# LanaSina/evolutionary_illusion_generator

Hardware: AMD Instinct MI355X
Metric: genome fitness evals/sec at 256x256, pop=256 (higher is better)
Workload: dtype f32; 1 GPU; neat_configs/circles.txt colour pop=256, 256x256, PredNet 3,48,96,192, 21 steps, LK + rotation-symmetry score; global_pop=256, genomes_per_gpu=256, device_batch=256, structure=Circles

## Files before the change

evolutionary_illusion_generator_amd/csrc/conv_mfma.h:

```cpp
#pragma once
#include <hip/hip_runtime.h>
#include <stdint.h>

#include <type_traits>

#ifndef EIG_PRO_PRIO
#define EIG_PRO_PRIO 1
#endif
#ifndef EIG_EPI_PRIO
#define EIG_EPI_PRIO 0
#endif
#ifndef EIG_KLOOP_PRIO
#define EIG_KLOOP_PRIO 0
#endif
#ifndef EIG_S8
#define EIG_S8 16
#endif
#ifndef EIG_ABLATE
#define EIG_ABLATE 0
#endif

namespace eig {

typedef float f32x4 __attribute__((ext_vector_type(4)));

enum { EPI_RAW = 0, EPI_LSTM = 1, EPI_CONVA = 2, EPI_CONVP = 3, EPI_LSTM_PACKED = 4, EPI_UP4 = 5, EPI_UP4C = 6 };
constexpr int epi_taps(int epi) { return (epi == EPI_UP4 || epi == EPI_UP4C) ? 4 : 9; }

struct ConvSrc {
    const float* ptr;
    int C;
    int Cpad;
    int _reserved;
    int Ct;
};

struct ConvArgs {
    ConvSrc src[3];
    int nsrc;
    int H, W, B;
    int tilesX, tilesY;
    int n_nblk;
    int nwalk, nparts;
    unsigned mg[3];
    int krows;
    const float* wpk;
    int Cout;
    int clip;
    const float* bias;
    float* c_state;
    float* h_out;
    const float* peep;
    const float* P;
    float* E;
    float* Pout;
    const uint8_t* img;
    long long img_bstride;
    float* E0;
    uint8_t* frame;
    long long frame_bstride;
    int requant;
    int tile_map;
    float* raw;
    const float* acc_init;
    const float* up_src;
    int up_C;
    int up_kb;
    const float* zeros;
    unsigned long long* dbg;
};

__device__ __forceinline__ float det_expf_core(float x)
{
    const float n = rintf(x * 1.44269504088896341f);
    float r = fmaf(n, -0.693359375f, x);
    r = fmaf(n, 2.12194440e-4f, r);
    float p = 1.9875691500e-4f;
    p = fmaf(p, r, 1.3981999507e-3f);
    p = fmaf(p, r, 8.3334519073e-3f);
    p = fmaf(p, r, 4.1665795894e-2f);
    p = fmaf(p, r, 1.6666665459e-1f);
    p = fmaf(p, r, 5.0000001201e-1f);
    const float r2 = r * r;
    const float y = fmaf(p, r2, r) + 1.0f;
    const float s = __int_as_float(((int)n + 127) << 23);
    return y * s;
}
__device__ __forceinline__ float det_expf(float x)
{
    x = fminf(x, 80.0f);
    x = fmaxf(x, -80.0f);
    return det_expf_core(x);
}
#ifndef EIG_GATE_ORDER
#define EIG_GATE_ORDER 1
#endif
__device__ __forceinline__ float det_tanhf(float x);
#if EIG_GATE_ORDER
__device__ __forceinline__ float det_sigmoidf(float x) { return det_tanhf(x * 0.5f) * 0.5f + 0.5f; }
#else
__device__ __forceinline__ float det_sigmoidf(float x) { return 1.0f / (1.0f + det_expf(-x)); }
#endif
__device__ __forceinline__ float det_tanhf(float x)
{
    float ax = fabsf(x);
    if (ax < 0.625f) {
        const float z = x * x;
        float p = -5.70498872745e-3f;
        p = fmaf(p, z, 2.06390887954e-2f);
        p = fmaf(p, z, -5.37397155531e-2f);
        p = fmaf(p, z, 1.33314422036e-1f);
        p = fmaf(p, z, -3.33332819422e-1f);
        const float pz = p * z;
        return fmaf(pz, x, x);
    }
    ax = fminf(ax, 10.0f);
    const float t = det_expf_core(2.0f * ax);
    const float d = t + 1.0f, rc = __builtin_amdgcn_rcpf(d);
    float q = 2.0f * rc;
    q = fmaf(fmaf(-d, q, 2.0f), rc, q);
    const float r = 1.0f - q;
    return x < 0.0f ? -r : r;
}
__device__ __forceinline__ float relu_f(float v) { return v > 0.0f ? v : 0.0f; }

__device__ __forceinline__ void lstm_cell(float zi_, float zf_, float zc_, float zo_, float bi, float bf, float bc, float bo,
                                          float cold, float pi_, float pf_, float po_, float& cn, float& hn)
{
#if EIG_GATE_ORDER
    const float zi = (zi_ + bi) + pi_ * cold;
    const float zf = (zf_ + bf) + pf_ * cold;
    const float zc = zc_ + bc;
    const float zo = (zo_ + bo) + po_ * cold;
    const float ii = det_sigmoidf(zi), ff = det_sigmoidf(zf), oo = det_sigmoidf(zo);
    float cc = det_tanhf(zc);
    cc = cc * ii;
    const float fc = ff * cold;
    cn = cc + fc;
    hn = oo * det_tanhf(cn);
#else
    float zi = zi_ + bi; zi = fmaf(pi_, cold, zi);
    float zf = zf_ + bf; zf = fmaf(pf_, cold, zf);
    const float zc = zc_ + bc;
    float zo = zo_ + bo; zo = fmaf(po_, cold, zo);
    const float ii = det_sigmoidf(zi), ff = det_sigmoidf(zf), gg = det_tanhf(zc), oo = det_sigmoidf(zo);
    const float gi = gg * ii;
    cn = fmaf(ff, cold, gi);
    hn = oo * det_tanhf(cn);
#endif
}

template <int TW, bool VEC, bool HALF = false> struct TileGeom {
    static constexpr int TH = (TW == 8) ? 8 : 16;
    static constexpr int NIMG = HALF ? 2 : 256 / (TH * TW);
    static constexpr int S = VEC ? (TW == 16 ? TW + 8 : (TW == 4 ? 12 : EIG_S8)) : TW + 2;
    static constexpr int XO = VEC ? 3 : 0;
    static constexpr int PH = TH + 2;
    static constexpr int PLANE = NIMG * PH * S;
};

#ifndef EIG_DMA_EARLY
#define EIG_DMA_EARLY 0
#endif
#ifndef EIG_KC
#define EIG_KC 8
#endif
constexpr int KC = EIG_KC;

template <int NI, int TW, bool VEC> constexpr bool conv_fast_dma() { return VEC && TW == 16 && KC == 8 && NI >= 3; }
template <int NI, int TW, bool VEC, int TAPS = 9, int NT = 256> constexpr int conv_w_floats()
{
    return (conv_fast_dma<NI, TW, VEC>() && !(NI == 4 && TAPS == 9)) ? ((KC * TAPS * NI * 4 + NT - 1) / NT) * NT * 4 : KC * TAPS * NI * 16;
}
template <int NI, int TW, bool VEC, int NT = 256, bool HALF = false> constexpr int conv_in_floats()
{
    return conv_fast_dma<NI, TW, VEC>() ? ((KC * TileGeom<TW, VEC>::PLANE / 4 + NT - 1) / NT) * NT * 4 : KC * TileGeom<TW, VEC, HALF>::PLANE;
}
template <int NI, int TW, bool VEC, int TAPS = 9, bool ONEKB = false, int NT = 256, bool HALF = false> constexpr int conv_lds_bytes()
{
    return (ONEKB ? 1 : 2) * (conv_in_floats<NI, TW, VEC, NT, HALF>() + conv_w_floats<NI, TW, VEC, TAPS, NT>()) * 4;
}

#ifndef EIG_TIMING
#define EIG_TIMING 0
#endif
#ifndef EIG_CONV_OCC
#define EIG_CONV_OCC 2
#endif
constexpr int CONV_THREADS = 256;
#ifndef EIG_W8_OCC
#define EIG_W8_OCC 4
#endif

#ifndef EIG_UP4_OCC
#define EIG_UP4_OCC 2
#endif
#ifndef EIG_ONEKB_OCC
#define EIG_ONEKB_OCC 4
#endif
template <int NI, int TW, int EPI, bool VEC, bool ONEKB = false, bool FUSE_ = false, int SPLIT = 0>
__global__ void __launch_bounds__(SPLIT == 1 ? 512 : CONV_THREADS, SPLIT ? EIG_W8_OCC : (ONEKB ? EIG_ONEKB_OCC : ((EPI == EPI_UP4 && NI == 4 && TW == 16 && VEC) ? EIG_UP4_OCC : EIG_CONV_OCC)))
conv3x3_mfma(const ConvArgs a)
{
    constexpr bool W8 = SPLIT != 0;
    constexpr bool H4 = SPLIT == 2;
    static_assert(!H4 || TW == 8 || TW == 4, "SPLIT 2: 8- or 4-wide tiles (one image per wave) only");
    static_assert(TW != 4 || (H4 && VEC && EPI != EPI_LSTM_PACKED && EPI != EPI_UP4C), "4-wide tiles: half blocks with 16-byte staging only");
    static_assert(!FUSE_, "the in-kernel chain of an unpooled source was removed in round 6 (a ConvLSTM chains it inside only in its Winograd forms)");
    static_assert(!W8 || (VEC && !ONEKB && EPI != EPI_UP4C && EPI != EPI_LSTM_PACKED), "W8: 16-byte staging, per-pixel or pooled epilogues");
    constexpr int NT = SPLIT == 1 ? 512 : CONV_THREADS;
    constexpr int NWS = H4 ? 2 : 4;
    constexpr int MI_N = W8 ? 2 : 4;
    using G = TileGeom<TW, VEC, H4>;
    constexpr int TH = G::TH, NIMG = G::NIMG, S = G::S, XO = G::XO, PH = G::PH, PLANE = G::PLANE;
    constexpr int NB = NI * 16;
    constexpr int TAPS = epi_taps(EPI);
    static_assert(EPI != EPI_UP4C || NI == 4, "EPI_UP4C: the four N-tiles are the four parity classes");
    const unsigned long long t_entry = EIG_TIMING ? __builtin_readcyclecounter() : 0;
#if EIG_PRO_PRIO
    __builtin_amdgcn_s_setprio(EIG_PRO_PRIO);
#endif
    extern __shared__ __attribute__((aligned(16))) float lds[];
    constexpr bool FAST = conv_fast_dma<NI, TW, VEC>();
    constexpr int INF = conv_in_floats<NI, TW, VEC, NT, H4>();
    constexpr int BUF = INF + conv_w_floats<NI, TW, VEC, epi_taps(EPI), NT>();

    const int tid = threadIdx.x;
    const int lane = tid & 63;
    const int wv = __builtin_amdgcn_readfirstlane(tid >> 6);
    const int ws = W8 ? (wv % NWS) : wv;
    const int ch2 = W8 ? (wv / NWS) : 0;
    const int q = lane >> 4;
    const int col = lane & 15;

    const int tiles = a.tilesX * a.tilesY;
    const int ngroups = (a.B + NIMG - 1) / NIMG;
    const int ntile = ngroups * tiles;
    const int xcd = blockIdx.x & 7, xi = blockIdx.x >> 3;
    const int nnb = (EPI == EPI_UP4) ? a.n_nblk * 4 : a.n_nblk;
    const int nbe = xi % nnb;
    const int nblk = (EPI == EPI_UP4) ? nbe >> 2 : nbe;
    const int cls = (EPI == EPI_UP4) ? nbe & 3 : 0;
    const int tlin = a.tile_map ? xcd * ((ntile + 7) >> 3) + xi / nnb : (xi / nnb) * 8 + xcd;
    if (tlin >= ntile) return;
    const int bgrp = tlin / tiles;
    const int t = tlin - bgrp * tiles;
    const int tyi = t / a.tilesX, txi = t - tyi * a.tilesX;
    const int y0 = tyi * TH, x0 = txi * TW;

    constexpr int RC = S / 4;
    constexpr int PER_C = VEC ? NIMG * PH * RC : PLANE;
    constexpr int NR = VEC ? (KC * PER_C + NT - 1) / NT : (PLANE + NT - 1) / NT;
    int sl_off[NR], sl_img[NR];
#pragma unroll
    for (int r = 0; r < NR; ++r) {
        const int p = tid + r * NT;
        int rem = VEC ? p % PER_C : p;
        constexpr int RW = VEC ? RC : S;
        const int img = rem / (PH * RW);
        rem -= img * (PH * RW);
        const int yy = rem / RW, xx = rem - yy * RW;
        const int gy = y0 + yy - 1, gx = VEC ? (x0 - 4 + 4 * xx) : (x0 + xx - 1);
        const int b = bgrp * NIMG + img;
        const bool ok = (VEC ? p < KC * PER_C : p < PLANE) && b < a.B && gy >= 0 && gy < a.H && gx >= 0 && gx < a.W;
        sl_off[r] = ok ? (VEC ? ((p / PER_C) * a.H * a.W + gy * a.W + gx) * 4 : gy * a.W + gx) : -1;
        sl_img[r] = VEC ? img : b;
    }

    constexpr int NWR = (KC * TAPS * (NB / 4) + NT - 1) / NT;
    constexpr int NIN = VEC ? NR : KC * NR;
    constexpr int NOPS = NWR + NIN;
    constexpr int NSTEP = KC * TAPS / 4;
    struct KB { int s, c0, kc; };
    const int cpad0 = a.src[0].Cpad, cpad1 = a.src[1].Cpad, cpad2 = a.src[2].Cpad;
    auto cpad_of = [&](int si) __attribute__((always_inline)) { return si == 0 ? cpad0 : (si == 1 ? cpad1 : cpad2); };
    auto kb_first = [&]() { KB k; k.s = 0; k.c0 = 0; k.kc = min(KC, cpad0); return k; };
    auto kb_next = [&](KB k) __attribute__((always_inline)) {
        k.c0 += KC;
        if (k.c0 >= cpad_of(k.s)) { k.c0 = 0; ++k.s; }
        k.kc = (k.s < a.nsrc) ? min(KC, cpad_of(k.s) - k.c0) : 0;
        return k;
    };
    const int b0 = bgrp * NIMG;
    const int nimg_here = min(NIMG, a.B - b0);
    auto make_rsrc = [&](const float* ptr, int C, int Ct) {
        const size_t plane = (size_t)(a.H * a.W);
        return __builtin_amdgcn_make_buffer_rsrc((void*)(ptr + (size_t)b0 * Ct * plane), 0, (int)(((size_t)(nimg_here - 1) * Ct + C) * plane * 4), 0x00020000);
    };
    const bool has1 = a.nsrc > 1, has2 = a.nsrc > 2;
    const __amdgpu_buffer_rsrc_t rs0 = make_rsrc(a.src[0].ptr, a.src[0].C, a.src[0].Ct);
    const __amdgpu_buffer_rsrc_t rs1 = make_rsrc(has1 ? a.src[1].ptr : a.src[0].ptr, has1 ? a.src[1].C : a.src[0].C, has1 ? a.src[1].Ct : a.src[0].Ct);
    const __amdgpu_buffer_rsrc_t rs2 = make_rsrc(has2 ? a.src[2].ptr : a.src[0].ptr, has2 ? a.src[2].C : a.src[0].C, has2 ? a.src[2].Ct : a.src[0].Ct);
    const __amdgpu_buffer_rsrc_t rsw = __builtin_amdgcn_make_buffer_rsrc((void*)(a.wpk + ((size_t)cls * a.n_nblk + nblk) * a.krows * NB), 0, a.krows * NB * 4, 0x00020000);
    auto buf_dma16 = [&](int si, float* lds_dst, int voff, int soff) {
        auto l = (__attribute__((address_space(3))) void*)lds_dst;
        if (si == 0) __builtin_amdgcn_raw_ptr_buffer_load_lds(rs0, l, 16, voff, soff, 0, 0);
        else if (si == 1) __builtin_amdgcn_raw_ptr_buffer_load_lds(rs1, l, 16, voff, soff, 0, 0);
        else __builtin_amdgcn_raw_ptr_buffer_load_lds(rs2, l, 16, voff, soff, 0, 0);
    };
    auto dma_op = [&](int j, const KB& k, int wrow, float* buf) {
        ConvSrc src;
        src.ptr = k.s == 0 ? a.src[0].ptr : (k.s == 1 ? a.src[1].ptr : a.src[2].ptr);
        src.C = k.s == 0 ? a.src[0].C : (k.s == 1 ? a.src[1].C : a.src[2].C);
        src.Cpad = cpad_of(k.s);
        src.Ct = k.s == 0 ? a.src[0].Ct : (k.s == 1 ? a.src[1].Ct : a.src[2].Ct);
        if (j < NWR) {
            const int n16 = k.kc * TAPS * (NB / 4);
            const int base = j * NT + wv * 64, ch = base + lane;
            if (ch < n16)
                __builtin_amdgcn_raw_ptr_buffer_load_lds(rsw, (__attribute__((address_space(3))) void*)(buf + INF + (size_t)base * 4), 16,
                                                         tid * 16, (wrow * NB + j * NT * 4) * 4, 0, 0);
            return;
        }
        const int chs = a.H * a.W;
        if (VEC) {
            const int r = j - NWR;
            const int p = tid + r * NT;
            const int soff = k.c0 * chs * 4;
            const bool tail = k.c0 + KC > src.C;
            if (r < NR) {
                int vo = sl_off[r < NR ? r : 0];
                if (NIMG > 1) vo = vo < 0 ? vo : vo + sl_img[r < NR ? r : 0] * src.Ct * chs * 4;
                if (tail && k.c0 + p / PER_C >= src.C) vo = -1;
                if (p < k.kc * PER_C) buf_dma16(k.s, buf + (r * NT + wv * 64) * 4, vo, soff);
            }
        } else {
            const int c = (j - NWR) / NR, r = (j - NWR) % NR;
            if (c < k.kc) {
                const bool pok = sl_off[r] >= 0;
                const int gy = pok ? sl_off[r] / a.W : 0, gx = pok ? sl_off[r] - gy * a.W : 0;
                const float* g = (pok && (k.c0 + c < src.C))
                                     ? src.ptr + ((size_t)sl_img[r] * src.Ct + k.c0 + c) * chs + gy * a.W + gx : a.zeros;
                if (tid + r * NT < PLANE)
                    __builtin_amdgcn_global_load_lds((const __attribute__((address_space(1))) void*)g,
                                                     (__attribute__((address_space(3))) void*)(buf + c * PLANE + r * NT + wv * 64), 4, 0, 0);
            }
        }
    };

    constexpr int LASTW = (NWR - 1) * NT;
    const int vw_full = tid * 16;
    const int vw_last = (LASTW + (wv & 1) * 64 + lane) * 16;
    static_assert(!FAST || NI != 4 || TAPS != 9 || (KC * 9 * (NB / 4)) % NT == 128, "FAST staging: the last weight round of NI = 4 must hold 128 chunks");
    static_assert(!FAST || TAPS != 4 || NI != 4 || (KC * 4 * (NB / 4)) % NT == 0, "FAST staging, 2x2 form: whole weight rounds");
    const int aH = a.H, aW = a.W;
    auto src_base = [&](const float* ptr, int Ct) __attribute__((always_inline)) { return ptr + (size_t)b0 * Ct * (a.H * a.W); };
    auto src_bytes = [&](int C, int Ct) __attribute__((always_inline)) { return ((nimg_here - 1) * Ct + C) * (a.H * a.W) * 4; };
    const float* const sp0 = src_base(a.src[0].ptr, a.src[0].Ct);
    const float* const sp1 = has1 ? src_base(a.src[1].ptr, a.src[1].Ct) : sp0;
    const float* const sp2 = has2 ? src_base(a.src[2].ptr, a.src[2].Ct) : sp0;
    const int sn0 = src_bytes(a.src[0].C, a.src[0].Ct);
    const int sn1 = has1 ? src_bytes(a.src[1].C, a.src[1].Ct) : sn0;
    const int sn2 = has2 ? src_bytes(a.src[2].C, a.src[2].Ct) : sn0;
    const unsigned long long su0 = (unsigned long long)sp0, sd1 = (unsigned long long)sp1 - su0, sd2 = (unsigned long long)sp2 - (unsigned long long)sp1;
    auto rsrc_of = [=](int si) __attribute__((always_inline)) {
        const unsigned long long u = su0 + (si > 0 ? sd1 : 0ull) + (si > 1 ? sd2 : 0ull);
        const int n = sn0 + (si > 0 ? sn1 - sn0 : 0) + (si > 1 ? sn2 - sn1 : 0);
        const unsigned lo = __builtin_amdgcn_readfirstlane((unsigned)u), hi = __builtin_amdgcn_readfirstlane((unsigned)(u >> 32));
        return __builtin_amdgcn_make_buffer_rsrc((void*)(((unsigned long long)hi << 32) | lo), 0, __builtin_amdgcn_readfirstlane(n), 0x00020000);
    };
    auto dma_fast = [=](int j, const KB k, const __amdgpu_buffer_rsrc_t rs_k, unsigned soff_in, unsigned soff_w, float* buf) __attribute__((always_inline)) {
        if (j < NWR) {
            const unsigned soff = soff_w;
            const bool lastw = TAPS == 9 && NI == 4 && (j == NWR - 1);
            if (SPLIT == 1 && lastw && wv >= 2) return;
            const unsigned vo = __builtin_elementwise_add_sat((unsigned)(lastw ? vw_last : vw_full + j * NT * 16), soff);
            float* dst = buf + INF + (lastw ? (LASTW + (wv & 1) * 64) * 4 : (j * NT + wv * 64) * 4);
            __builtin_amdgcn_raw_ptr_buffer_load_lds(rsw, (__attribute__((address_space(3))) void*)dst, 16, (int)vo, 0, 0, 0);
            return;
        }
        const int r = j - NWR;
        const unsigned soff = soff_in;
        const int slot = r < NR ? sl_off[r < NR ? r : 0] : -1;
        const unsigned vo = __builtin_elementwise_add_sat((unsigned)slot, soff);
        __builtin_amdgcn_raw_ptr_buffer_load_lds(rs_k, (__attribute__((address_space(3))) void*)(buf + (r * NT + wv * 64) * 4), 16, (int)vo, 0, 0, 0);
    };

    const unsigned long long t_setup = EIG_TIMING ? __builtin_readcyclecounter() : 0;
    int nkb = 0;
    for (int s = 0; s < a.nsrc; ++s) nkb += (cpad_of(s) + KC - 1) / KC;
    KB cur_kb = kb_first();
    int wrow = 0;

#pragma unroll
    for (int j = 0; j < NOPS; ++j) {
        if constexpr (FAST) dma_fast(j, cur_kb, rsrc_of(0), 0u, 0u, lds);
        else dma_op(j, cur_kb, wrow, lds);
    }

    int addrA[9];
    const int g_wy = (TW == 16) ? (col & 3) >> 1 : (TW == 4 ? 2 * (col >> 2) + ((col & 3) >> 1) : col >> 2);
    const int g_wx = (TW == 16) ? 2 * (col >> 2) + (col & 1) : (TW == 4 ? col & 1 : col & 3);
    const int g_base = ((TW == 16) ? (ws * 4 + 2 * g_wy) * S + 2 * g_wx + XO
                                   : ws * PH * S + 2 * g_wy * S + 2 * g_wx + XO)
                       + ch2 * S;
    {
#pragma unroll
        for (int s = 0; s < 9; ++s) {
            const int k = 4 * s + q;
            const int c = k / 9, tap = k - 9 * c;
            const int ky = tap / 3, kx = tap - 3 * ky;
            addrA[s] = g_base + c * PLANE + ky * S + kx;
        }
    }
    const int addr4 = g_base + ((q >> 1) + (cls >> 1)) * S + (q & 1) + (cls & 1);
    const int boff = q * NB + col * NI;

    f32x4 acc[MI_N][NI];
#pragma unroll
    for (int mi = 0; mi < MI_N; ++mi)
#pragma unroll
        for (int ni = 0; ni < NI; ++ni) acc[mi][ni] = (f32x4){0.f, 0.f, 0.f, 0.f};

    const unsigned long long t_prewait = EIG_TIMING ? __builtin_readcyclecounter() : 0;
#if EIG_KLOOP_PRIO
    __builtin_amdgcn_s_setprio(EIG_KLOOP_PRIO);
#endif
#if EIG_PRO_PRIO
    __builtin_amdgcn_s_setprio(0);
#endif
    asm volatile("s_waitcnt vmcnt(0)" ::: "memory");
    __syncthreads();

    constexpr bool HAS_UP = (EPI == EPI_LSTM || EPI == EPI_LSTM_PACKED || EPI == EPI_RAW);
    constexpr int UPV = (TW != 8) ? 2 : 1;
    constexpr int NUPL = HAS_UP ? MI_N * NI * UPV : 0;
    f32x4 upc[MI_N][HAS_UP ? NI : 1];
    const bool has_up = HAS_UP && a.acc_init != nullptr;
    int up_off[UPV];
    const float* up_base = a.acc_init;
    int up_hw = 0, up_cstride = 0;
    if (has_up) {
        const int Hs = a.H >> 1, Ws = a.W >> 1;
        up_hw = Hs * Ws;
        up_cstride = a.n_nblk * NB * up_hw;
        const int b = bgrp * NIMG + (TW == 16 ? 0 : ws);
#pragma unroll
        for (int v = 0; v < UPV; ++v) {
            const int gy0 = (TW == 16) ? y0 + 4 * ws + 2 * v : (TW == 4 ? tyi * TH + 4 * q + 2 * v : tyi * TH + 2 * q);
            const int gx0 = (TW == 16) ? x0 + 4 * q : txi * TW;
            up_off[v] = (b < a.B && gy0 < a.H && gx0 < a.W) ? ((nblk * NB + col) * up_hw + (gy0 >> 1) * Ws + (gx0 >> 1)) * 4 : 0;
        }
        const int bw = __builtin_amdgcn_readfirstlane(b);
        up_base = a.acc_init + (size_t)(bw < a.B ? bw : 0) * 4 * up_cstride;
    }
    const __amdgpu_buffer_rsrc_t rs_up = __builtin_amdgcn_make_buffer_rsrc((void*)up_base, 0, has_up ? 4 * up_cstride * 4 : 0, 0x00020000);
    auto up_load = [&](int mi, int ni, int v) __attribute__((always_inline)) {
        const int soff = (ni * 16 * up_hw + (W8 ? 2 * ch2 + mi : mi) * up_cstride) * 4;
        if constexpr (TW != 8) {
            typedef float f32x2 __attribute__((ext_vector_type(2)));
            const f32x2 t = __builtin_bit_cast(f32x2, __builtin_amdgcn_raw_buffer_load_b64(rs_up, up_off[v], soff, 0));
            upc[mi][ni][2 * v] = t[0]; upc[mi][ni][2 * v + 1] = t[1];
        } else {
            upc[mi][ni] = __builtin_bit_cast(f32x4, __builtin_amdgcn_raw_buffer_load_b128(rs_up, up_off[0], soff, 0));
        }
    };

    unsigned long long t_mfma = 0, t_wait = 0, t_bar = 0, t_all0 = EIG_TIMING ? __builtin_readcyclecounter() : 0;
    auto kiter = [&](const int kb, auto kfirst_tag) __attribute__((always_inline)) {
        const unsigned long long tk0 = EIG_TIMING ? __builtin_readcyclecounter() : 0;
        float* const cur = lds + (kb & 1) * BUF;
        float* const nxt = lds + ((kb & 1) ^ 1) * BUF;
        const KB nxt_kb = kb_next(cur_kb);
        const int wrow_nxt = wrow + cur_kb.kc * TAPS;
        const bool more_kb = (kb + 1 < nkb) && EIG_ABLATE != 1;
        const __amdgpu_buffer_rsrc_t rs_nxt = rsrc_of(nxt_kb.s);
        const unsigned soff_in_nxt = more_kb ? (unsigned)(nxt_kb.c0 * (aH * aW) * 4) : 0x80000000u;
        const unsigned soff_w_nxt = more_kb ? (unsigned)(wrow_nxt * NB * 4) : 0x80000000u;

        const float* const in_lds = cur;
        const float* const w_lds = cur + INF + boff;
        auto body = [&](auto first_tag) {
            constexpr bool FIRST = decltype(first_tag)::value;
            constexpr int PL = PLANE;
            const int* const ad = addrA;
#pragma unroll
            for (int st = 0; st < NSTEP; ++st) {
                if (FAST || (TAPS == 9 ? (st < 9 || cur_kb.kc > 4) : st < cur_kb.kc)) {
                    const int per = st / 9, s9 = st % 9;
                    float av[MI_N], bv[NI];
                    float avc[MI_N][3];
#pragma unroll
                    for (int mi = 0; mi < MI_N; ++mi) {
                        const int moff = W8 ? mi : (mi >> 1) * S + (mi & 1);
                        av[mi] = (TAPS == 9) ? in_lds[ad[s9] + per * 4 * PL + moff] : in_lds[addr4 + st * PL + moff];
                        if constexpr (EPI == EPI_UP4C) {
#pragma unroll
                            for (int c = 1; c < 4; ++c) avc[mi][c - 1] = in_lds[addr4 + ((c >> 1) * S + (c & 1)) + st * PL + moff];
                        }
                    }
                    if (NI == 4) {
                        const f32x4 b4 = *reinterpret_cast<const f32x4*>(w_lds + st * 4 * NB);
#pragma unroll
                        for (int ni = 0; ni < NI; ++ni) bv[ni] = b4[ni];
                    } else {
#pragma unroll
                        for (int ni = 0; ni < NI; ++ni) bv[ni] = w_lds[st * 4 * NB + ni];
                    }
#pragma unroll
                    for (int mi = 0; mi < MI_N; ++mi)
#pragma unroll
                        for (int ni = 0; ni < NI; ++ni)
                            acc[mi][ni] = __builtin_amdgcn_mfma_f32_16x16x4f32((EPI == EPI_UP4C && ni > 0) ? avc[mi][ni > 0 ? ni - 1 : 0] : av[mi], bv[ni], acc[mi][ni], 0, 0, 0);
                }
                if constexpr (ONEKB) {
                } else if constexpr (FAST) {
#pragma unroll
                    for (int j = 0; j < NOPS; ++j)
                        if ((EIG_DMA_EARLY ? (j * EIG_DMA_EARLY < NSTEP ? j * EIG_DMA_EARLY : NSTEP - 1) : j * NSTEP / NOPS) == st) dma_fast(j, nxt_kb, rs_nxt, soff_in_nxt, soff_w_nxt, nxt);
                } else if (more_kb) {
#pragma unroll
                    for (int j = 0; j < NOPS; ++j)
                        if (j * NSTEP / NOPS == st) dma_op(j, nxt_kb, wrow_nxt, nxt);
                }
                if constexpr (FIRST) {
#pragma unroll
                    for (int mi = 0; mi < MI_N; ++mi)
#pragma unroll
                        for (int ni = 0; ni < NI; ++ni)
#pragma unroll
                            for (int v = 0; v < UPV; ++v)
                                if (((mi * NI + ni) * UPV + v) * NSTEP / NUPL == st) up_load(mi, ni, v);
                    __builtin_amdgcn_sched_barrier(0);
                }
            }
        };
        body(kfirst_tag);
        wrow = wrow_nxt;
        cur_kb = nxt_kb;
        const unsigned long long tk1 = EIG_TIMING ? __builtin_readcyclecounter() : 0;
        asm volatile("s_waitcnt vmcnt(0)" ::: "memory");
        const unsigned long long tk2 = EIG_TIMING ? __builtin_readcyclecounter() : 0;
        __syncthreads();
        if (EIG_TIMING) { const unsigned long long tk3 = __builtin_readcyclecounter(); t_mfma += tk1 - tk0; t_wait += tk2 - tk1; t_bar += tk3 - tk2; }
    };
    int kb_begin = 0;
    if constexpr (HAS_UP) {
        if (has_up) { kiter(0, std::true_type{}); kb_begin = 1; }
    }
    for (int kb = kb_begin; kb < nkb; ++kb) kiter(kb, std::false_type{});
#if EIG_KLOOP_PRIO
    __builtin_amdgcn_s_setprio(0);
#endif
#if EIG_EPI_PRIO
    __builtin_amdgcn_s_setprio(EIG_EPI_PRIO);
#endif
    const unsigned long long t_loop1 = EIG_TIMING ? __builtin_readcyclecounter() : 0;

    if (has_up) {
#pragma unroll
        for (int mi = 0; mi < MI_N; ++mi)
#pragma unroll
            for (int ni = 0; ni < (HAS_UP ? NI : 1); ++ni) acc[mi][ni] = acc[mi][ni] + upc[mi][ni];
    }
    const int HW = a.H * a.W;
    auto timeline_record = [&](unsigned long long t_mid) {
        if (EIG_TIMING && a.dbg && lane == 0) {
            unsigned hwid, xcc;
            asm volatile("s_getreg_b32 %0, hwreg(HW_REG_HW_ID)" : "=s"(hwid));
            asm volatile("s_getreg_b32 %0, hwreg(HW_REG_XCC_ID)" : "=s"(xcc));
            unsigned long long* d = a.dbg + ((size_t)blockIdx.x * (W8 ? 8 : 4) + wv) * 8;
            d[0] = t_entry; d[1] = t_all0; d[2] = t_loop1; d[3] = __builtin_readcyclecounter();
            d[4] = (unsigned long long)hwid | ((unsigned long long)xcc << 32); d[5] = t_mfma; d[6] = t_setup; d[7] = t_prewait; (void)t_mid; (void)t_bar;
        }
    };
    typedef float f32x2 __attribute__((ext_vector_type(2)));
    const int eb = bgrp * NIMG + (TW == 16 ? 0 : ws);
    const int ey0 = (TW == 16) ? y0 + 4 * ws : tyi * TH;
    const int ex0 = (TW == 16) ? x0 : txi * TW;
    auto seg_row = [&](int sgi) __attribute__((always_inline)) { return ey0 + ((TW == 16) ? sgi : (TW == 4 ? 4 * q + sgi : 2 * q + (sgi >> 1))); };
    auto seg_col = [&](int sgi) __attribute__((always_inline)) { return ex0 + ((TW == 16) ? 4 * q : (TW == 4 ? 0 : 4 * (sgi & 1))); };
    constexpr int NSEG = W8 ? 2 : 4;
#define EIG_SGI(sl) (W8 ? ((TW != 8) ? ch2 + 2 * (sl) : 2 * ch2 + (sl)) : (sl))
#define EIG_SEG_MI(sl, j) (W8 ? ((j) & 1) : ((TW != 8) ? 2 * ((sl) & 1) + ((j) & 1) : 2 * ((sl) >> 1) + ((j) & 1)))
#define EIG_SEG_REG(sl, j) (W8 ? 2 * (sl) + ((j) >> 1) : ((TW != 8) ? 2 * ((sl) >> 1) + ((j) >> 1) : 2 * ((sl) & 1) + ((j) >> 1)))
    const bool alive = eb < a.B;
    if (!alive && !(W8 && EPI == EPI_CONVA)) { timeline_record(0); return; }

    if constexpr (EPI == EPI_RAW || EPI == EPI_UP4 || EPI == EPI_UP4C) {
#pragma unroll
        for (int ni = 0; ni < NI; ++ni) {
            float* dst;
            if (EPI == EPI_UP4C) {
                if ((col & 3) >= a.Cout) continue;
                dst = a.raw + (((size_t)eb * 4 + ni) * a.n_nblk * 16 + nblk * 16 + col) * HW;
            }
            else if (EPI == EPI_UP4) dst = a.raw + (((size_t)eb * 4 + cls) * a.n_nblk * NB + nblk * NB + ni * 16 + col) * HW;
            else {
                const int o = nblk * NB + ni * 16 + col;
                if (o >= a.Cout) continue;
                dst = a.raw + ((size_t)eb * a.Cout + o) * HW;
            }
#pragma unroll
            for (int sgi = 0; sgi < NSEG; ++sgi) {
                const int gy = seg_row(EIG_SGI(sgi)), gx = seg_col(EIG_SGI(sgi));
                if (gy >= a.H || gx >= a.W) continue;
                if (VEC) {
                    *reinterpret_cast<f32x4*>(dst + gy * a.W + gx) = (f32x4){acc[EIG_SEG_MI(sgi, 0)][ni][EIG_SEG_REG(sgi, 0)], acc[EIG_SEG_MI(sgi, 1)][ni][EIG_SEG_REG(sgi, 1)],
                                                                              acc[EIG_SEG_MI(sgi, 2)][ni][EIG_SEG_REG(sgi, 2)], acc[EIG_SEG_MI(sgi, 3)][ni][EIG_SEG_REG(sgi, 3)]};
                    continue;
                }
#pragma unroll
                for (int j = 0; j < 4; ++j)
                    if (gx + j < a.W) dst[gy * a.W + gx + j] = acc[EIG_SEG_MI(sgi, j)][ni][EIG_SEG_REG(sgi, j)];
            }
        }
    } else if constexpr (EPI == EPI_LSTM) {
        const int ch = nblk * 16 + col;
        if (ch < a.Cout) {
            const float bi = a.bias[ch], bf = a.bias[a.Cout + ch], bc = a.bias[2 * a.Cout + ch], bo = a.bias[3 * a.Cout + ch];
            const size_t cbase = ((size_t)eb * a.Cout + ch) * HW;
            const size_t pbase = (size_t)ch * HW;
            const size_t pstride = (size_t)a.Cout * HW;
            auto cell = [&](float zi_, float zf_, float zc_, float zo_, float cold, float pi_, float pf_, float po_, float& cn, float& hn) __attribute__((always_inline)) {
                if (EIG_ABLATE == 2) { cn = (zi_ + bi) + (zf_ + bf) + pi_ * cold; hn = (zc_ + bc) + (zo_ + bo) + pf_ * po_; return; }
                lstm_cell(zi_, zf_, zc_, zo_, bi, bf, bc, bo, cold, pi_, pf_, po_, cn, hn);
            };
#pragma unroll
            for (int sgi = 0; sgi < NSEG; ++sgi) {
                const int gy = seg_row(EIG_SGI(sgi)), gx = seg_col(EIG_SGI(sgi));
                if (gy >= a.H || gx >= a.W) continue;
                const int pix = gy * a.W + gx;
                if (VEC) {
                    const f32x4 cold4 = *reinterpret_cast<const f32x4*>(a.c_state + cbase + pix);
                    const f32x4 pi4 = *reinterpret_cast<const f32x4*>(a.peep + pbase + pix);
                    const f32x4 pf4 = *reinterpret_cast<const f32x4*>(a.peep + pstride + pbase + pix);
                    const f32x4 po4 = *reinterpret_cast<const f32x4*>(a.peep + 2 * pstride + pbase + pix);
                    f32x4 cn4, hn4;
#pragma unroll
                    for (int j = 0; j < 4; ++j) {
                        float cn, hn;
                        cell(acc[EIG_SEG_MI(sgi, j)][0][EIG_SEG_REG(sgi, j)], acc[EIG_SEG_MI(sgi, j)][1][EIG_SEG_REG(sgi, j)], acc[EIG_SEG_MI(sgi, j)][2][EIG_SEG_REG(sgi, j)],
                             acc[EIG_SEG_MI(sgi, j)][3][EIG_SEG_REG(sgi, j)], cold4[j], pi4[j], pf4[j], po4[j], cn, hn);
                        cn4[j] = cn; hn4[j] = hn;
                    }
                    *reinterpret_cast<f32x4*>(a.c_state + cbase + pix) = cn4;
                    *reinterpret_cast<f32x4*>(a.h_out + cbase + pix) = hn4;
                    continue;
                }
#pragma unroll
                for (int j = 0; j < 4; ++j) {
                    if (gx + j >= a.W) continue;
                    float cn, hn;
                    cell(acc[EIG_SEG_MI(sgi, j)][0][EIG_SEG_REG(sgi, j)], acc[EIG_SEG_MI(sgi, j)][1][EIG_SEG_REG(sgi, j)], acc[EIG_SEG_MI(sgi, j)][2][EIG_SEG_REG(sgi, j)],
                         acc[EIG_SEG_MI(sgi, j)][3][EIG_SEG_REG(sgi, j)], a.c_state[cbase + pix + j], a.peep[pbase + pix + j], a.peep[pstride + pbase + pix + j],
                         a.peep[2 * pstride + pbase + pix + j], cn, hn);
                    a.c_state[cbase + pix + j] = cn;
                    a.h_out[cbase + pix + j] = hn;
                }
            }
        }
    } else if constexpr (EPI == EPI_LSTM_PACKED) {
        const int ch = col & 3, g = col >> 2;
        const bool active = ch < a.Cout;
        const int cc = active ? ch : 0;
#pragma unroll
        for (int mi = 0; mi < 4; ++mi) {
            float r[4];
#pragma unroll
            for (int d = 0; d < 4; ++d) {
                const int sel = (g + d) & 3;
                const float v = sel == 0 ? acc[mi][0][0] : (sel == 1 ? acc[mi][0][1] : (sel == 2 ? acc[mi][0][2] : acc[mi][0][3]));
                r[d] = (d == 0) ? v : __shfl(v, (lane & ~12) | (((g - d) & 3) << 2), 64);
            }
            auto gate = [&](int sg) {
                const int d = (g - sg) & 3;
                return d == 0 ? r[0] : (d == 1 ? r[1] : (d == 2 ? r[2] : r[3]));
            };
            const float ai = gate(0), af = gate(1), ac = gate(2), ao = gate(3);
            const int gy = ey0 + ((TW == 16) ? 2 * (g >> 1) + (mi >> 1) : 2 * q + (mi >> 1));
            const int gx = ex0 + ((TW == 16) ? 4 * q + 2 * (g & 1) + (mi & 1) : 2 * g + (mi & 1));
            if (!active || gy >= a.H || gx >= a.W) continue;
            const float bi = a.bias[cc], bf = a.bias[a.Cout + cc], bc = a.bias[2 * a.Cout + cc], bo = a.bias[3 * a.Cout + cc];
            const size_t cbase = ((size_t)eb * a.Cout + cc) * HW;
            const size_t pbase = (size_t)cc * HW;
            const size_t pstride = (size_t)a.Cout * HW;
            const int pix = gy * a.W + gx;
            const float cold = a.c_state[cbase + pix];
            float cnew, hnew;
            lstm_cell(ai, af, ac, ao, bi, bf, bc, bo, cold, a.peep[pbase + pix], a.peep[pstride + pbase + pix], a.peep[2 * pstride + pbase + pix], cnew, hnew);
            a.c_state[cbase + pix] = cnew;
            a.h_out[cbase + pix] = hnew;
        }
    } else if constexpr (EPI == EPI_CONVA) {
        const int Ho = a.H >> 1, Wo = a.W >> 1;
        const size_t plane = (size_t)Ho * Wo;
        constexpr int NPR = (TW != 8) ? 2 : 1, NPC = (TW != 8) ? 2 : 4;
        const int pyo = (ey0 >> 1) + ((TW == 16) ? 0 : (TW == 4 ? 2 * q : q)), pxo = (ex0 >> 1) + ((TW == 16) ? 2 * q : 0);
        const bool vec_ok = VEC && (TW != 8 || (a.W % 8) == 0);
        float* const xch = lds;
        if constexpr (W8) {
            __syncthreads();
#pragma unroll
            for (int ni = 0; ni < NI; ++ni) {
                const int chx = nblk * NB + ni * 16 + col;
                const float bbx = chx < a.Cout ? a.bias[chx] : 0.0f;
#pragma unroll
                for (int reg = 0; reg < 4; ++reg)
                    xch[((wv * NI + ni) * 4 + reg) * 64 + lane] = fmaxf(relu_f(acc[0][ni][reg] + bbx), relu_f(acc[1][ni][reg] + bbx));
            }
            __syncthreads();
            if (!alive) { timeline_record(0); return; }
        }
#pragma unroll
        for (int ni = 0; ni < NI; ++ni) {
            const int ch = nblk * NB + ni * 16 + col;
            if (ch >= a.Cout) continue;
            if (W8 && TW == 8 && NI > 1 && (ni & 1) != ch2) continue;
            if (W8 && TW == 8 && NI == 1 && ch2 != 0) continue;
            const float bb = a.bias[ch];
            float A[4];
#pragma unroll
            for (int reg = 0; reg < 4; ++reg) {
                if constexpr (W8) {
                    const float m0 = xch[(((ws) * NI + ni) * 4 + reg) * 64 + lane], m1 = xch[(((ws + NWS) * NI + ni) * 4 + reg) * 64 + lane];
                    A[reg] = fmaxf(m0, m1);
                } else {
                    const float v0 = relu_f(acc[0][ni][reg] + bb), v1 = relu_f(acc[1][ni][reg] + bb);
                    const float v2 = relu_f(acc[MI_N - 2][ni][reg] + bb), v3 = relu_f(acc[MI_N - 1][ni][reg] + bb);
                    A[reg] = fmaxf(fmaxf(v0, v1), fmaxf(v2, v3));
                }
            }
            const float* Pc = a.P + ((size_t)eb * a.Cout + ch) * plane;
            float* Ec = a.E + ((size_t)eb * 2 * a.Cout + ch) * plane;
            float* Ec2 = Ec + (size_t)a.Cout * plane;
#pragma unroll
            for (int pr = 0; pr < NPR; ++pr) {
                if (W8 && TW != 8 && pr != ch2) continue;
                const int yo = pyo + pr;
                if (yo >= Ho || pxo >= Wo) continue;
                const size_t o = (size_t)yo * Wo + pxo;
                if (vec_ok) {
                    if constexpr (TW != 8) {
                        const f32x2 p2 = *reinterpret_cast<const f32x2*>(Pc + o);
                        const float A0 = A[2 * pr], A1 = A[2 * pr + 1];
                        *reinterpret_cast<f32x2*>(Ec + o) = (f32x2){relu_f(A0 - p2[0]), relu_f(A1 - p2[1])};
                        *reinterpret_cast<f32x2*>(Ec2 + o) = (f32x2){relu_f(p2[0] - A0), relu_f(p2[1] - A1)};
                    } else {
                        const f32x4 p4 = *reinterpret_cast<const f32x4*>(Pc + o);
                        *reinterpret_cast<f32x4*>(Ec + o) = (f32x4){relu_f(A[0] - p4[0]), relu_f(A[1] - p4[1]), relu_f(A[2] - p4[2]), relu_f(A[3] - p4[3])};
                        *reinterpret_cast<f32x4*>(Ec2 + o) = (f32x4){relu_f(p4[0] - A[0]), relu_f(p4[1] - A[1]), relu_f(p4[2] - A[2]), relu_f(p4[3] - A[3])};
                    }
                    continue;
                }
#pragma unroll
                for (int pc = 0; pc < NPC; ++pc) {
                    if (pxo + pc >= Wo) continue;
                    const float Av = A[(TW != 8) ? 2 * pr + pc : pc];
                    const float p = Pc[o + pc];
                    Ec[o + pc] = relu_f(Av - p);
                    Ec2[o + pc] = relu_f(p - Av);
                }
            }
        }
    } else if constexpr (EPI == EPI_CONVP) {
#pragma unroll
        for (int ni = 0; ni < NI; ++ni) {
            const int ch = nblk * NB + ni * 16 + col;
            if (ch >= a.Cout) continue;
            const float bb = a.bias[ch];
            const size_t base = ((size_t)eb * a.Cout + ch) * HW;
#pragma unroll
            for (int sgi = 0; sgi < NSEG; ++sgi) {
                const int gy = seg_row(EIG_SGI(sgi)), gx = seg_col(EIG_SGI(sgi));
                if (gy >= a.H || gx >= a.W) continue;
                const int pix = gy * a.W + gx;
                if (VEC && !a.frame && !a.E0) {
                    f32x4 v4;
#pragma unroll
                    for (int j = 0; j < 4; ++j) {
                        float v = relu_f(acc[EIG_SEG_MI(sgi, j)][ni][EIG_SEG_REG(sgi, j)] + bb);
                        if (a.clip) v = fminf(v, 1.0f);
                        v4[j] = v;
                    }
                    *reinterpret_cast<f32x4*>(a.Pout + base + pix) = v4;
                    continue;
                }
#pragma unroll
                for (int j = 0; j < 4; ++j) {
                    if (gx + j >= a.W) continue;
                    float v = relu_f(acc[EIG_SEG_MI(sgi, j)][ni][EIG_SEG_REG(sgi, j)] + bb);
                    if (a.clip) v = fminf(v, 1.0f);
                    a.Pout[base + pix + j] = v;
                    if (a.frame) a.frame[(size_t)eb * a.frame_bstride + (size_t)ch * HW + pix + j] = (uint8_t)(int)(v * 255.0f);
                    if (a.E0) {
                        float x;
                        if (a.img) x = (float)a.img[(size_t)eb * a.img_bstride + (size_t)ch * HW + pix + j] / 255.0f;
                        else if (a.requant) x = (float)(uint8_t)(int)(v * 255.0f) / 255.0f;
                        else x = v;
                        const size_t e = ((size_t)eb * 2 * a.Cout + ch) * HW + pix + j;
                        a.E0[e] = relu_f(x - v);
                        a.E0[e + (size_t)a.Cout * HW] = relu_f(v - x);
                    }
                }
            }
        }
    }
#undef EIG_SGI
#undef EIG_SEG_MI
#undef EIG_SEG_REG
    timeline_record(0);
}

constexpr int P0_TX = 64, P0_TY = 8;
template <int C>
__global__ void __launch_bounds__(P0_TX * P0_TY) convp0_direct_kernel(const float* __restrict__ src, const float* __restrict__ wgt ,
                                                                     const ConvArgs a)
{
    __shared__ float tile[C][P0_TY + 2][P0_TX + 2];
    const int tx = threadIdx.x & (P0_TX - 1), ty = threadIdx.x / P0_TX;
    const int x0 = blockIdx.x * P0_TX, y0 = blockIdx.y * P0_TY, b = blockIdx.z;
    const int HW = a.H * a.W;
    const float* sb = src + (size_t)b * C * HW;
    for (int i = threadIdx.x; i < C * (P0_TY + 2) * (P0_TX + 2); i += P0_TX * P0_TY) {
        const int c = i / ((P0_TY + 2) * (P0_TX + 2));
        const int r = i - c * ((P0_TY + 2) * (P0_TX + 2));
        const int yy = r / (P0_TX + 2), xx = r - yy * (P0_TX + 2);
        const int gy = y0 + yy - 1, gx = x0 + xx - 1;
        tile[c][yy][xx] = (gy >= 0 && gy < a.H && gx >= 0 && gx < a.W) ? sb[(size_t)c * HW + gy * a.W + gx] : 0.0f;
    }
    __syncthreads();
    const int gy = y0 + ty, gx = x0 + tx;
    if (gy >= a.H || gx >= a.W) return;
    const int pix = gy * a.W + gx;
#pragma unroll
    for (int o = 0; o < C; ++o) {
        float acc = 0.0f;
#pragma unroll
        for (int c = 0; c < C; ++c)
#pragma unroll
            for (int ky = 0; ky < 3; ++ky)
#pragma unroll
                for (int kx = 0; kx < 3; ++kx) acc = fmaf(tile[c][ty + ky][tx + kx], wgt[((o * C + c) * 3 + ky) * 3 + kx], acc);
        const size_t base = ((size_t)b * C + o) * HW;
        float v = relu_f(acc + a.bias[o]);
        if (a.clip) v = fminf(v, 1.0f);
        a.Pout[base + pix] = v;
        if (a.frame) a.frame[(size_t)b * a.frame_bstride + (size_t)o * HW + pix] = (uint8_t)(int)(v * 255.0f);
        if (a.E0) {
            float x;
            if (a.img) x = (float)a.img[(size_t)b * a.img_bstride + (size_t)o * HW + pix] / 255.0f;
            else if (a.requant) x = (float)(uint8_t)(int)(v * 255.0f) / 255.0f;
            else x = v;
            const size_t e = ((size_t)b * 2 * C + o) * HW + pix;
            a.E0[e] = relu_f(x - v);
            a.E0[e + (size_t)C * HW] = relu_f(v - x);
        }
    }
}

constexpr int L0_TX = 64, L0_TY = 8;
template <int C, bool T0>
__global__ void __launch_bounds__(L0_TX * L0_TY) lstm0_direct_kernel(const float* __restrict__ srcE, const float* __restrict__ srcH,
                                                                    const float* __restrict__ wgt, const ConvArgs a)
{
    constexpr int CE = T0 ? C : 2 * C, CH = T0 ? 0 : C;
    constexpr int K = (CE + CH) * 9;
    __shared__ float tile[CE + (CH ? CH : 1)][L0_TY + 2][L0_TX + 2];
    const int tx = threadIdx.x & (L0_TX - 1), ty = threadIdx.x / L0_TX;
    const int x0 = blockIdx.x * L0_TX, y0 = blockIdx.y * L0_TY, b = blockIdx.z;
    const int HW = a.H * a.W;
    constexpr int PLANE = (L0_TY + 2) * (L0_TX + 2);
    for (int i = threadIdx.x; i < (CE + CH) * PLANE; i += L0_TX * L0_TY) {
        const int c = i / PLANE;
        const int r = i - c * PLANE;
        const int yy = r / (L0_TX + 2), xx = r - yy * (L0_TX + 2);
        const int gy = y0 + yy - 1, gx = x0 + xx - 1;
        float v = 0.0f;
        if (gy >= 0 && gy < a.H && gx >= 0 && gx < a.W)
            v = (c < CE) ? srcE[((size_t)b * 2 * C + c) * HW + gy * a.W + gx] : srcH[((size_t)b * C + (c - CE)) * HW + gy * a.W + gx];
        tile[c][yy][xx] = v;
    }
    __syncthreads();
    const int gy = y0 + ty, gx = x0 + tx;
    if (gy >= a.H || gx >= a.W) return;
    const int pix = gy * a.W + gx;
    const f32x4* const w4 = reinterpret_cast<const f32x4*>(wgt) + (T0 ? C * (3 * C * 9) : 0);
    const int Hs = a.H >> 1, Ws = a.W >> 1;
    const size_t up_hw = (size_t)Hs * Ws;
    const float* up = a.acc_init ? a.acc_init + (((size_t)b * 4 + ((gy & 1) * 2 + (gx & 1))) * 16) * up_hw + (size_t)(gy >> 1) * Ws + (gx >> 1) : nullptr;
#pragma unroll
    for (int o = 0; o < C; ++o) {
        float z[4] = {0.0f, 0.0f, 0.0f, 0.0f};
#pragma unroll
        for (int c = 0; c < CE + CH; ++c)
#pragma unroll
            for (int ky = 0; ky < 3; ++ky)
#pragma unroll
                for (int kx = 0; kx < 3; ++kx) {
                    const float v = tile[c][ty + ky][tx + kx];
                    const f32x4 w = w4[o * K + (c * 3 + ky) * 3 + kx];
#pragma unroll
                    for (int g = 0; g < 4; ++g) z[g] = fmaf(v, w[g], z[g]);
                }
        if (up) {
#pragma unroll
            for (int g = 0; g < 4; ++g) z[g] = z[g] + up[(size_t)(g * 4 + o) * up_hw];
        }
        const float bi = a.bias[o], bf = a.bias[C + o], bc = a.bias[2 * C + o], bo = a.bias[3 * C + o];
        const size_t cbase = ((size_t)b * C + o) * HW;
        const size_t pbase = (size_t)o * HW;
        const size_t pstride = (size_t)C * HW;
        const float cold = a.c_state[cbase + pix];
        float cnew, hnew;
        lstm_cell(z[0], z[1], z[2], z[3], bi, bf, bc, bo, cold, a.peep[pbase + pix], a.peep[pstride + pbase + pix], a.peep[2 * pstride + pbase + pix], cnew, hnew);
        a.c_state[cbase + pix] = cnew;
        a.h_out[cbase + pix] = hnew;
    }
}

#ifdef EIG_ENGINE_UNIT
__global__ void e0_init_kernel(const uint8_t* img, long long img_bstride, float* E0, int C, int HW, int B)
{
    const size_t n = (size_t)B * C * HW;
    for (size_t i = blockIdx.x * (size_t)blockDim.x + threadIdx.x; i < n; i += (size_t)gridDim.x * blockDim.x) {
        const size_t b = i / ((size_t)C * HW);
        const size_t r = i - b * (size_t)C * HW;
        const float x = (float)img[b * img_bstride + r] / 255.0f;
        E0[b * 2 * C * HW + r] = relu_f(x - 0.0f);
        E0[b * 2 * C * HW + (size_t)C * HW + r] = relu_f(0.0f - x);
    }
}

__global__ void e0_resume_kernel(const float* P0, const uint8_t* img, long long img_bstride, int requant, float* E0, int C, int HW, int B)
{
    const size_t n = (size_t)B * C * HW;
    for (size_t i = blockIdx.x * (size_t)blockDim.x + threadIdx.x; i < n; i += (size_t)gridDim.x * blockDim.x) {
        const size_t b = i / ((size_t)C * HW);
        const size_t r = i - b * (size_t)C * HW;
        const float v = P0[i];
        float x;
        if (img) x = (float)img[b * img_bstride + r] / 255.0f;
        else if (requant) x = (float)(uint8_t)(int)(v * 255.0f) / 255.0f;
        else x = v;
        E0[b * 2 * C * HW + r] = relu_f(x - v);
        E0[b * 2 * C * HW + (size_t)C * HW + r] = relu_f(v - x);
    }
}

__global__ void det_math_kernel(const float* x, int n, float* e, float* s, float* t)
{
    const int i = blockIdx.x * blockDim.x + threadIdx.x;
    if (i < n) {
        if (e) e[i] = det_expf(x[i]);
        if (s) s[i] = det_sigmoidf(x[i]);
        if (t) t[i] = det_tanhf(x[i]);
    }
}
#endif

}
```

Before: 429.4 genome evals/s.

## Vectorise lstm0 tile staging, pack FMAs, add CONVA row-order finishing path

The lstm0 direct kernel now stages its halo tile with 16-byte loads into a wider padded shared-memory row. Its 4-gate accumulation uses packed two-wide FMAs, which could map to packed-FP32 instructions. In the conv kernel, new compile-time options add an image-order epilogue for the CONVA error layer, a prefetch of the prediction tile before the K loop, and skipping of zero K-steps. These are off by default except the prefetch, which only runs when the off-by-default row-order path is enabled. Together they aim to cut scalar global loads and FMA issue count, at the cost of extra LDS padding and more code paths.

Result: no change. 431.4 genome evals/s (median of 6 runs) (+0.5%).

```diff
diff --git a/evolutionary_illusion_generator_amd/csrc/conv_mfma.h b/evolutionary_illusion_generator_amd/csrc/conv_mfma.h
--- a/evolutionary_illusion_generator_amd/csrc/conv_mfma.h
+++ b/evolutionary_illusion_generator_amd/csrc/conv_mfma.h
@@ -198,6 +198,16 @@
 #ifndef EIG_ONEKB_OCC
 #define EIG_ONEKB_OCC 4
 #endif
+#ifndef EIG_CONVA_ROWFIN
+#define EIG_CONVA_ROWFIN 0
+#endif
+#ifndef EIG_CONVA_PFETCH
+#define EIG_CONVA_PFETCH 1
+#endif
+#ifndef EIG_CONVA_SKIPZ
+#define EIG_CONVA_SKIPZ 0
+#endif
+constexpr int ROWFIN_CS = 72;
 template <int NI, int TW, int EPI, bool VEC, bool ONEKB = false, bool FUSE_ = false, int SPLIT = 0>
 __global__ void __launch_bounds__(SPLIT == 1 ? 512 : CONV_THREADS, SPLIT ? EIG_W8_OCC : (ONEKB ? EIG_ONEKB_OCC : ((EPI == EPI_UP4 && NI == 4 && TW == 16 && VEC) ? EIG_UP4_OCC : EIG_CONV_OCC)))
 conv3x3_mfma(const ConvArgs a)
@@ -419,6 +429,25 @@
 #if EIG_PRO_PRIO
     __builtin_amdgcn_s_setprio(0);
 #endif
+    constexpr bool ROWFIN = EIG_CONVA_ROWFIN && EPI == EPI_CONVA && ONEKB && TW == 16 && VEC && !W8;
+    constexpr int RF_N = ROWFIN ? NB * 16 / NT : 1;
+    static_assert(!ROWFIN || (NB * ROWFIN_CS * 4 <= conv_lds_bytes<NI, TW, VEC, TAPS, ONEKB, NT, H4>() && (NB * 16) % NT == 0), "image-order finishing: the pooled tile must fit the K-block's buffer");
+    bool rowfin = false;
+    f32x4 rf_p[RF_N];
+    if constexpr (ROWFIN) {
+        rowfin = (a.W & 7) == 0 && x0 + TW <= a.W && y0 + TH <= a.H;
+        if (EIG_CONVA_PFETCH && rowfin) {
+            const int Wo = a.W >> 1;
+            const size_t plane = (size_t)(a.H >> 1) * Wo;
+#pragma unroll
+            for (int r = 0; r < RF_N; ++r) {
+                const int chl = (tid >> 4) + 16 * r, jj = ((tid & 15) - 2 * chl) & 15;
+                const int ch = nblk * NB + chl;
+                rf_p[r] = (f32x4){0.0f, 0.0f, 0.0f, 0.0f};
+                if (ch < a.Cout) rf_p[r] = *reinterpret_cast<const f32x4*>(a.P + ((size_t)b0 * a.Cout + ch) * plane + (size_t)((y0 >> 1) + (jj >> 1)) * Wo + (x0 >> 1) + 4 * (jj & 1));
+            }
+        }
+    }
     asm volatile("s_waitcnt vmcnt(0)" ::: "memory");
     __syncthreads();
 
@@ -476,7 +505,8 @@
             const int* const ad = addrA;
 #pragma unroll
             for (int st = 0; st < NSTEP; ++st) {
-                if (FAST || (TAPS == 9 ? (st < 9 || cur_kb.kc > 4) : st < cur_kb.kc)) {
+                if (EIG_CONVA_SKIPZ && ONEKB && EPI == EPI_CONVA && st * 4 >= a.src[0].C * TAPS) {
+                } else if (FAST || (TAPS == 9 ? (st < 9 || cur_kb.kc > 4) : st < cur_kb.kc)) {
                     const int per = st / 9, s9 = st % 9;
                     float av[MI_N], bv[NI];
                     float avc[MI_N][3];
@@ -702,6 +732,42 @@
             __syncthreads();
             if (!alive) { timeline_record(0); return; }
         }
+        if constexpr (ROWFIN) {
+            if (rowfin) {
+#pragma unroll
+                for (int ni = 0; ni < NI; ++ni) {
+                    const int ch = nblk * NB + ni * 16 + col;
+                    const float bb = ch < a.Cout ? a.bias[ch] : 0.0f;
+                    float A[4];
+#pragma unroll
+                    for (int reg = 0; reg < 4; ++reg) {
+                        const float v0 = relu_f(acc[0][ni][reg] + bb), v1 = relu_f(acc[1][ni][reg] + bb);
+                        const float v2 = relu_f(acc[2][ni][reg] + bb), v3 = relu_f(acc[3][ni][reg] + bb);
+                        A[reg] = fmaxf(fmaxf(v0, v1), fmaxf(v2, v3));
+                    }
+#pragma unroll
+                    for (int pr = 0; pr < 2; ++pr)
+                        *reinterpret_cast<f32x2*>(xch + (ni * 16 + col) * ROWFIN_CS + (2 * ws + pr) * 8 + 2 * q) = (f32x2){A[2 * pr], A[2 * pr + 1]};
+                }
+                __syncthreads();
+                const size_t plane = (size_t)Ho * Wo;
+#pragma unroll
+                for (int r = 0; r < RF_N; ++r) {
+                    const int chl = (tid >> 4) + 16 * r, jj = ((tid & 15) - 2 * chl) & 15;
+                    const int ch = nblk * NB + chl;
+                    if (ch >= a.Cout) continue;
+                    const f32x4 A4 = *reinterpret_cast<const f32x4*>(xch + chl * ROWFIN_CS + jj * 4);
+                    const size_t o = (size_t)((y0 >> 1) + (jj >> 1)) * Wo + (x0 >> 1) + 4 * (jj & 1);
+                    const f32x4 p4 = EIG_CONVA_PFETCH ? rf_p[r] : *reinterpret_cast<const f32x4*>(a.P + ((size_t)eb * a.Cout + ch) * plane + o);
+                    float* Ec = a.E + ((size_t)eb * 2 * a.Cout + ch) * plane;
+                    if (EIG_ABLATE == 3 && A4[0] != 12345.678f) continue;
+                    *reinterpret_cast<f32x4*>(Ec + o) = (f32x4){relu_f(A4[0] - p4[0]), relu_f(A4[1] - p4[1]), relu_f(A4[2] - p4[2]), relu_f(A4[3] - p4[3])};
+                    *reinterpret_cast<f32x4*>(Ec + (size_t)a.Cout * plane + o) = (f32x4){relu_f(p4[0] - A4[0]), relu_f(p4[1] - A4[1]), relu_f(p4[2] - A4[2]), relu_f(p4[3] - A4[3])};
+                }
+                timeline_record(0);
+                return;
+            }
+        }
 #pragma unroll
         for (int ni = 0; ni < NI; ++ni) {
             const int ch = nblk * NB + ni * 16 + col;
@@ -849,27 +915,55 @@
     }
 }
 
+#ifndef EIG_L0_PACKED
+#define EIG_L0_PACKED 1
+#endif
+#ifndef EIG_L0_WIDE
+#define EIG_L0_WIDE 1
+#endif
 constexpr int L0_TX = 64, L0_TY = 8;
+constexpr int L0_S = EIG_L0_WIDE ? L0_TX + 8 : L0_TX + 2, L0_XO = EIG_L0_WIDE ? 3 : 0;
 template <int C, bool T0>
 __global__ void __launch_bounds__(L0_TX * L0_TY) lstm0_direct_kernel(const float* __restrict__ srcE, const float* __restrict__ srcH,
                                                                     const float* __restrict__ wgt, const ConvArgs a)
 {
+    typedef float f32x2 __attribute__((ext_vector_type(2)));
     constexpr int CE = T0 ? C : 2 * C, CH = T0 ? 0 : C;
     constexpr int K = (CE + CH) * 9;
-    __shared__ float tile[CE + (CH ? CH : 1)][L0_TY + 2][L0_TX + 2];
+    __shared__ __attribute__((aligned(16))) float tile[CE + (CH ? CH : 1)][L0_TY + 2][L0_S];
     const int tx = threadIdx.x & (L0_TX - 1), ty = threadIdx.x / L0_TX;
     const int x0 = blockIdx.x * L0_TX, y0 = blockIdx.y * L0_TY, b = blockIdx.z;
     const int HW = a.H * a.W;
-    constexpr int PLANE = (L0_TY + 2) * (L0_TX + 2);
-    for (int i = threadIdx.x; i < (CE + CH) * PLANE; i += L0_TX * L0_TY) {
-        const int c = i / PLANE;
-        const int r = i - c * PLANE;
-        const int yy = r / (L0_TX + 2), xx = r - yy * (L0_TX + 2);
-        const int gy = y0 + yy - 1, gx = x0 + xx - 1;
-        float v = 0.0f;
-        if (gy >= 0 && gy < a.H && gx >= 0 && gx < a.W)
-            v = (c < CE) ? srcE[((size_t)b * 2 * C + c) * HW + gy * a.W + gx] : srcH[((size_t)b * C + (c - CE)) * HW + gy * a.W + gx];
-        tile[c][yy][xx] = v;
+    if (EIG_L0_WIDE && (a.W & 3) == 0) {
+        constexpr int RC = L0_S / 4, PER_C = (L0_TY + 2) * RC;
+        constexpr int NCH = (CE + CH) * PER_C, NT = L0_TX * L0_TY;
+#pragma unroll
+        for (int r = 0; r < (NCH + NT - 1) / NT; ++r) {
+            const int i = threadIdx.x + r * NT;
+            if (i >= NCH) continue;
+            const int c = i / PER_C;
+            const int rem = i - c * PER_C;
+            const int yy = rem / RC, xc = rem - yy * RC;
+            const int gy = y0 + yy - 1, gx = x0 - 4 + 4 * xc;
+            f32x4 v = (f32x4){0.0f, 0.0f, 0.0f, 0.0f};
+            if (gy >= 0 && gy < a.H && gx >= 0 && gx < a.W) {
+                const float* p = (c < CE) ? srcE + ((size_t)b * 2 * C + c) * HW : srcH + ((size_t)b * C + (c - CE)) * HW;
+                v = *reinterpret_cast<const f32x4*>(p + gy * a.W + gx);
+            }
+            *reinterpret_cast<f32x4*>(&tile[c][yy][4 * xc]) = v;
+        }
+    } else {
+        constexpr int PLANE = (L0_TY + 2) * (L0_TX + 2);
+        for (int i = threadIdx.x; i < (CE + CH) * PLANE; i += L0_TX * L0_TY) {
+            const int c = i / PLANE;
+            const int r = i - c * PLANE;
+            const int yy = r / (L0_TX + 2), xx = r - yy * (L0_TX + 2);
+            const int gy = y0 + yy - 1, gx = x0 + xx - 1;
+            float v = 0.0f;
+            if (gy >= 0 && gy < a.H && gx >= 0 && gx < a.W)
+                v = (c < CE) ? srcE[((size_t)b * 2 * C + c) * HW + gy * a.W + gx] : srcH[((size_t)b * C + (c - CE)) * HW + gy * a.W + gx];
+            tile[c][yy][xx + L0_XO] = v;
+        }
     }
     __syncthreads();
     const int gy = y0 + ty, gx = x0 + tx;
@@ -882,17 +976,24 @@
 #pragma unroll
     for (int o = 0; o < C; ++o) {
         float z[4] = {0.0f, 0.0f, 0.0f, 0.0f};
+        f32x2 zif = (f32x2){0.0f, 0.0f}, zco = (f32x2){0.0f, 0.0f};
 #pragma unroll
         for (int c = 0; c < CE + CH; ++c)
 #pragma unroll
             for (int ky = 0; ky < 3; ++ky)
 #pragma unroll
                 for (int kx = 0; kx < 3; ++kx) {
-                    const float v = tile[c][ty + ky][tx + kx];
+                    const float v = tile[c][ty + ky][tx + kx + L0_XO];
                     const f32x4 w = w4[o * K + (c * 3 + ky) * 3 + kx];
+                    if (EIG_L0_PACKED) {
+                        zif = __builtin_elementwise_fma((f32x2){v, v}, (f32x2){w[0], w[1]}, zif);
+                        zco = __builtin_elementwise_fma((f32x2){v, v}, (f32x2){w[2], w[3]}, zco);
+                        continue;
+                    }
 #pragma unroll
                     for (int g = 0; g < 4; ++g) z[g] = fmaf(v, w[g], z[g]);
                 }
+        if (EIG_L0_PACKED) { z[0] = zif[0]; z[1] = zif[1]; z[2] = zco[0]; z[3] = zco[1]; }
         if (up) {
 #pragma unroll
             for (int g = 0; g < 4; ++g) z[g] = z[g] + up[(size_t)(g * 4 + o) * up_hw];
```
